# thomasgilgenast/hic3defdr

Measured on AMD Instinct MI355X. Metric: pixels/sec through estimate_disp+lrt, 4 reps @10kb; max-|Δq| vs reference, higher is better.
Workload: dtype f64; 1 GPU; cfg2: per GPU 1 chrom x 20000 bins, 4 reps (2+2), dist_thresh_max 250, estimate_disp (qcml) + lrt on HBM-resident inputs; disp_pixels_rank0=3757837, disp_pixels_total=3757837, parallelism=dp1 (chromosome shards; in-kernel Brent searches)

## Files before the change

hic3defdr_amd/csrc/h3d_api.hip:

```cpp
#include <hip/hip_runtime.h>
#include <hipcub/hipcub.hpp>

#include <algorithm>
#include <chrono>
#include <cstdarg>
#include <cstdio>
#include <cstdlib>
#include <cstring>
#include <map>
#include <string>
#include <thread>
#include <vector>

#include "h3d.h"
#include "h3d_ctx.h"
#include "h3d_errors.h"
#include "h3d_host.h"
#include "h3d_kernels.h"

using namespace h3d;
using namespace h3dint;
using h3derr::fail;

namespace h3dint {
// ... 137 lines not shown
}

}

namespace {

struct HostStamps {
  bool on = std::getenv("H3D_TIMING") != nullptr;
  std::chrono::steady_clock::time_point t0 = std::chrono::steady_clock::now();
  void operator()(const char* what) const {
    if (on)
      fprintf(stderr, "[h3d timing] %8.1f us %s\n",
              std::chrono::duration<double, std::micro>(
                  std::chrono::steady_clock::now() - t0).count(), what);
  }
};

template <typename K>
int resident_blocks(K kernel) {
  int nb = 0;
  if (hipOccupancyMaxActiveBlocksPerMultiprocessor(&nb, kernel, kBlock, 0) != hipSuccess ||
      nb < 1)
    nb = 1;
  return nb;
}

template <typename K>
int work_grid(h3d_ctx* ctx, K kernel, size_t max_items) {
  int& nb = ctx->resident[(const void*)kernel];
  if (nb == 0) nb = resident_blocks(kernel);
  return (int)std::max<size_t>(1, std::min<size_t>(max_items, (size_t)ctx->n_cu * nb));
}

template <int M, bool NLL>
void launch_disp_work(h3d_ctx* ctx, size_t max_items, const int32_t* raw_s,
                      const double* f_s, double* pd, int64_t n,
                      const int64_t* cs, const int32_t* cl, const int32_t* cd,
                      int C, const int32_t* rep_idx, const int32_t* n_rep,
                      const SegState* st, int* seg_flags, const int32_t* list,
                      int32_t* meta, double* partial) {
  {
    ProfScope ps(ctx, "disp_work", 0, 1);
#define H3D_EQ(WW)                                                                  \
  do {                                                                              \
    auto k = k_disp_work<M, WW, kEqualize, NLL>;                                    \
    hipLaunchKernelGGL(k, dim3(work_grid(ctx, k, max_items)), dim3(kBlock), 0,      \
                       ctx->stream, raw_s, f_s, pd, n, cs, cl, cd, C, rep_idx, n_rep, \
                       st, seg_flags, list, meta, partial, ctx->eq_static8);        \
  } while (0)
    if constexpr (M == 2 && NLL) {
      H3D_EQ(4);
    } else if constexpr (M == 2) {
      if (ctx->disp_w2 == 8) H3D_EQ(8);
      else if (ctx->disp_w2 == 6) H3D_EQ(6);
      else if (ctx->disp_w2 == 5) H3D_EQ(5);
      else H3D_EQ(4);
    } else if constexpr (M == 4) {
      if (ctx->disp_w == 4) H3D_EQ(4);
      else if (ctx->disp_w == 3) H3D_EQ(3);
      else if (ctx->disp_w == 2) H3D_EQ(2);
      else H3D_EQ(1);
    } else if constexpr (M == 8) {
      if (ctx->disp_w8 == 4) H3D_EQ(4);
      else H3D_EQ(1);
    } else {
      H3D_EQ(1);
    }
#undef H3D_EQ
  }
  if constexpr (NLL) {
    ProfScope ps(ctx, "disp_nll", 0);
    auto k = k_disp_work<M, 1, kNll>;
    if constexpr (M == 4) {
      if (ctx->nll_w == 2) k = k_disp_work<M, 2, kNll>;
      else if (ctx->nll_w == 4) k = k_disp_work<M, 4, kNll>;
    }
    hipLaunchKernelGGL(k, dim3(work_grid(ctx, k, max_items)), dim3(kBlock), 0,
                       ctx->stream, raw_s, f_s, pd, n, cs, cl, cd, C, rep_idx, n_rep,
                       st, seg_flags, list, meta, partial, ctx->eq_static8);
  }
}

template <int M>
void launch_brent(h3d_ctx* ctx, const double* pd, int64_t n, const int64_t* seg_start,
                  int S, int C, const int32_t* rep_idx, const int32_t* n_rep,
                  SegState* st, const int* seg_flags, double* result, int* queue,
                  const int32_t* gate_meta = nullptr, int live_min = 0,
                  const int* gang_abort = nullptr, bool queue_zeroed = false) {
  ProfScope ps(ctx, "disp_nll", 0);
  auto k = k_brent<M>;
  constexpr int kBrentBlock = brent_block<M>();
  const size_t lds_max = M <= 8 ? (size_t)ctx->brent_lds_kb * 1024 : 0;
  int& nb = ctx->resident[(const void*)k];
  if (nb == 0) {
    if (lds_max)
      (void)hipFuncSetAttribute((const void*)k, hipFuncAttributeMaxDynamicSharedMemorySize,
                                (int)lds_max);
    if (hipOccupancyMaxActiveBlocksPerMultiprocessor(&nb, k, kBrentBlock, lds_max) !=
            hipSuccess ||
        nb < 1)
      nb = 1;
  }
  const int grid = std::max(1, std::min(S, ctx->n_cu * nb));
  const size_t lds_bytes = M <= 8 ? (size_t)ctx->brent_lds_kb * 1024 : 0;
  const int64_t lds_px = (int64_t)(lds_bytes / (8 * (size_t)M));
  if (!queue_zeroed) (void)hipMemsetAsync(queue, 0, sizeof(int), ctx->stream);
  hipLaunchKernelGGL(k, dim3(grid), dim3(kBrentBlock), lds_px ? lds_px * 8 * M : 0,
                     ctx->stream, pd, n, seg_start, S, C, rep_idx, n_rep, st, seg_flags,
                     result, queue, ctx->work_count, lds_px, gate_meta, live_min, gang_abort);
#ifdef H3D_BRENT_CLOCK
  unsigned long long clk[38];
  (void)hipMemcpyFromSymbolAsync(clk, HIP_SYMBOL(g_brent_clk), sizeof(clk), 0,
                                 hipMemcpyDeviceToHost, ctx->stream);
  (void)hipStreamSynchronize(ctx->stream);
  fprintf(stderr, "[brent_clk] sum %llu bar1 %llu step %llu bar2 %llu stage %llu total %llu\n",
          clk[0], clk[1], clk[2], clk[3], clk[4], clk[5]);
  fprintf(stderr, "[brent_clk_wave] sum");
  for (int i = 0; i < 16; ++i) fprintf(stderr, " %llu", clk[6 + i]);
  fprintf(stderr, " bar1");
  for (int i = 0; i < 16; ++i) fprintf(stderr, " %llu", clk[22 + i]);
  fprintf(stderr, "\n");
#endif
}

struct GangTables {
  int32_t* task_seg = nullptr;
  int32_t* task_g = nullptr;
  int T = 0, gmax = 1, grid = 0;
  int64_t P = 0;
  double* part = nullptr;
  int* tag = nullptr;
  int* abort = nullptr;
  long long timeout = 0;
};

int gang_next_epoch(h3d_ctx* ctx, const GangTables& g, int S) {
  const size_t cap = ctx->bufs["gang_tag"].second;
  if (ctx->gang_tag_buf != (void*)g.tag || ctx->gang_tag_cap != cap ||
// ... 75 lines not shown
}

template <int M>
int gang_setup_dev(h3d_ctx* ctx, int64_t n, int D, int C, GangTables* g) {
  auto k = k_brent_gang<M>;
  int& nb = ctx->resident[(const void*)k];
  if (nb == 0) {
    if (hipOccupancyMaxActiveBlocksPerMultiprocessor(&nb, k, kGangThreads, 0) != hipSuccess ||
        nb < 1)
      nb = 1;
  }
  g->grid = ctx->n_cu * nb;
  const int64_t total = n * C;
  int64_t P = (total + 2 * (int64_t)g->grid - 1) / (2 * (int64_t)g->grid);
  P = std::max<int64_t>(P, (n + g->grid - 1) / g->grid);
  P = std::max<int64_t>(1024, (P + kGangThreads - 1) / kGangThreads * kGangThreads);
  if (ctx->gang_px > 0)
    P = std::max<int64_t>(std::max<int64_t>(64, ctx->gang_px), (n + g->grid - 1) / g->grid);
  g->P = P;
  g->gmax = (int)std::max<int64_t>(1, (n + P - 1) / P);
  g->T = (int)std::min<int64_t>(INT32_MAX, (int64_t)C * (g->gmax + D));
  const int S = D * C;
  g->task_seg = (int32_t*)scratch(ctx, "gang_seg", (size_t)g->T * 4);
  g->task_g = (int32_t*)scratch(ctx, "gang_g", (size_t)g->T * 4);
  g->part = (double*)scratch(ctx, "gang_part", (size_t)2 * S * g->gmax * 8);
  g->tag = (int*)scratch(ctx, "gang_tag", (size_t)2 * S * g->gmax * 4);
  g->abort = (int*)scratch(ctx, "gang_abort", 4);
  if (!g->task_seg || !g->task_g || !g->part || !g->tag || !g->abort)
    return fail(H3D_ENOMEM, "gang tables");
  g->timeout = gang_timeout(ctx);
  return 0;
}

template <int M>
void launch_brent_gang(h3d_ctx* ctx, const double* pd, int64_t n, const int64_t* seg_start,
                       int S, int C, const int32_t* rep_idx, const int32_t* n_rep,
                       SegState* st, const int* seg_flags, double* result, int* queue,
                       const GangTables& g, const int32_t* gate_meta = nullptr,
                       int live_max = 0, bool queue_zeroed = false) {
  ProfScope ps(ctx, "disp_nll", 0);
  if (!queue_zeroed) (void)hipMemsetAsync(queue, 0, sizeof(int), ctx->stream);
  const int epoch = gang_next_epoch(ctx, g, S);
  const int grid = std::max(1, std::min(g.T, g.grid));
  hipLaunchKernelGGL(k_brent_gang<M>, dim3(grid), dim3(kGangThreads), 0, ctx->stream, pd,
                     n, seg_start, S, C, rep_idx, n_rep, st, seg_flags, result, queue,
                     g.task_seg, g.task_g, g.T, g.P, g.part, g.tag, g.gmax, g.abort,
                     g.timeout, ctx->work_count, epoch, gate_meta, live_max);
}

int64_t disp_work_bytes(h3d_ctx* ctx, bool nll) {
  unsigned long long c[2] = {0, 0};
  if (!ctx->work_count) return 0;
  (void)hipMemcpyAsync(c, ctx->work_count, sizeof(c), hipMemcpyDeviceToHost, ctx->stream);
  (void)hipStreamSynchronize(ctx->stream);
  return nll ? (int64_t)(c[1] * 8ull) : (int64_t)(c[0] * 20ull);
}

}

extern "C" {

int h3d_version(void) { return 1; }

const char* h3d_last_error(void) { return h3derr::last(); }

int h3d_device_count(void) {
  int n = 0;
  if (hipGetDeviceCount(&n) != hipSuccess) return 0;
  return n;
}

h3d_ctx* h3d_open(int device) {
  int n = 0;
  if (hipGetDeviceCount(&n) != hipSuccess || n == 0) {
    fail(H3D_ENODEV, "no HIP device visible");
    return nullptr;
  }
// ... 5 lines not shown
  if (hipGetDeviceProperties(&prop, device) != hipSuccess) {
    fail(H3D_EHIP, "hipGetDeviceProperties failed");
    return nullptr;
  }
  if (std::strncmp(prop.gcnArchName, "gfx950", 6) != 0) {
    fail(H3D_ENODEV, "device %d is %s, libh3d is built for gfx950", device,
         prop.gcnArchName);
    return nullptr;
  }
  if (hipSetDevice(device) != hipSuccess) {
    fail(H3D_EHIP, "hipSetDevice failed");
    return nullptr;
  }
  h3d_ctx* ctx = new h3d_ctx();
  ctx->device = device;
  ctx->n_cu = prop.multiProcessorCount;
  if (hipStreamCreateWithFlags(&ctx->own, hipStreamNonBlocking) != hipSuccess) {
    delete ctx;
    fail(H3D_EHIP, "stream create failed");
    return nullptr;
  }
  ctx->stream = ctx->own;
  if (const char* e = std::getenv("H3D_DISP_W")) ctx->disp_w = std::atoi(e);
  if (const char* e = std::getenv("H3D_DISP_SORT")) ctx->disp_sort = std::atoi(e);
  if (const char* e = std::getenv("H3D_NLL_W")) ctx->nll_w = std::atoi(e);
  if (const char* e = std::getenv("H3D_DISP_W8")) ctx->disp_w8 = std::atoi(e);
  if (const char* e = std::getenv("H3D_DISP_W2")) ctx->disp_w2 = std::atoi(e);
  if (const char* e = std::getenv("H3D_PACK_GATHER")) ctx->pack_gather = std::atoi(e);
  if (const char* e = std::getenv("H3D_EQ_STATIC8"))
    ctx->eq_static8 = std::max(0, std::min(8, std::atoi(e)));
  if (const char* e = std::getenv("H3D_DISP_M2")) ctx->disp_m2 = std::atoi(e);
  if (const char* e = std::getenv("H3D_BRENT")) ctx->brent_gang = std::atoi(e);
  if (const char* e = std::getenv("H3D_BRENT_LDS_KB")) ctx->brent_lds_kb = std::atoi(e);
  if (const char* e = std::getenv("H3D_GANG_P")) ctx->gang_px = std::atoi(e);
  if (const char* e = std::getenv("H3D_DEV_SEG_TABLES")) ctx->dev_seg_tables = std::atoi(e);
  if (hipMalloc((void**)&ctx->work_count, 2 * sizeof(unsigned long long)) != hipSuccess ||
      hipMemset(ctx->work_count, 0, 2 * sizeof(unsigned long long)) != hipSuccess) {
    (void)hipStreamDestroy(ctx->own);
    delete ctx;
    fail(H3D_ENOMEM, "counter allocation failed");
    return nullptr;
  }
  return ctx;
}

void h3d_close(h3d_ctx* ctx) {
  if (!ctx) return;
  (void)hipSetDevice(ctx->device);
  (void)hipStreamSynchronize(ctx->stream);
  prof_collect(ctx);
  for (auto& kv : ctx->bufs)
    if (kv.second.first) (void)hipFree(kv.second.first);
  for (auto e : ctx->event_pool) (void)hipEventDestroy(e);
  if (ctx->work_count) (void)hipFree(ctx->work_count);
  if (ctx->h_meta) (void)hipHostFree(ctx->h_meta);
  if (ctx->h_stage) (void)hipHostFree(ctx->h_stage);
  if (ctx->h_res) (void)hipHostFree(ctx->h_res);
  if (ctx->h_stage_done) (void)hipEventDestroy(ctx->h_stage_done);
  if (ctx->bounce) (void)hipHostFree(ctx->bounce);
  if (ctx->bounce_ev) (void)hipEventDestroy(ctx->bounce_ev);
  if (ctx->land) (void)hipHostFree(ctx->land);
  if (ctx->own) (void)hipStreamDestroy(ctx->own);
  delete ctx;
}

int h3d_set_stream(h3d_ctx* ctx, void* stream) {
// ... 369 lines not shown
  HIP_TRY(hipMemcpyAsync(d_blob + up_lo, (char*)ctx->h_stage + up_lo, up_hi - up_lo,
                         hipMemcpyHostToDevice, s));
  HIP_TRY(hipEventRecord(ctx->h_stage_done, s));
  int64_t* d_cs = (int64_t*)(d_blob + parts[0].off);
  int32_t* d_cl = (int32_t*)(d_blob + parts[1].off);
  int32_t* d_cd = (int32_t*)(d_blob + parts[2].off);
  int32_t* d_scb = (int32_t*)(d_blob + parts[3].off);
  int32_t* d_sce = (int32_t*)(d_blob + parts[4].off);
  int32_t* d_nrep = (int32_t*)(d_blob + parts[5].off);
  int32_t* d_repidx = (int32_t*)(d_blob + parts[6].off);
  SegState* d_st = (SegState*)(d_blob + parts[7].off);
  int64_t* d_lpx = (int64_t*)(d_blob + parts[8].off);
  const size_t max_items = (size_t)std::max(n_chunks, 1) * C;
  int32_t* d_list = (int32_t*)scratch(ctx, "work_list", max_items * 4);
  int32_t* d_meta = (int32_t*)scratch(ctx, "work_meta", kWorkMetaInts * 4);
  int32_t* d_slb = (int32_t*)scratch(ctx, "seg_lb", S * 4);
  int32_t* d_sle = (int32_t*)scratch(ctx, "seg_le", S * 4);
  double* d_partial = (double*)scratch(ctx, "partial", max_items * 8 * kWavesPerBlock);
  double* d_total = (double*)scratch(ctx, "seg_total", S * 8);
  int* d_flags = (int*)scratch(ctx, "seg_flags", S * 4);
  double* d_res = (double*)scratch(ctx, "seg_result", S * 8);
  if (!d_cs || !d_cl || !d_cd || !d_scb || !d_sce || !d_nrep || !d_repidx ||
      !d_st || !d_lpx || !d_list || !d_meta || !d_slb || !d_sle || !d_partial ||
      !d_total || !d_flags || !d_res)
    return fail(H3D_ENOMEM, "disp scratch");
  if (!dev_tables) HIP_TRY(hipMemsetAsync(d_flags, 0, S * 4, s));
  int* d_bad = (int*)scratch(ctx, "dist_bad", 4);
  if (!d_bad) return fail(H3D_ENOMEM, "dist_bad");
  const int mslot = (maxnr <= 2 && ctx->disp_m2) ? 2
                    : maxnr <= 4                  ? 4
                    : maxnr <= 8                  ? 8
                    : maxnr <= 16                 ? 16
                                                  : 32;
  GangTables gang;
  const bool dual = dev_tables && !reduce && ctx->brent_gang == 1;
  if (dual) {
    const int grc = mslot == 2    ? gang_setup_dev<2>(ctx, n, D, C, &gang)
                    : mslot == 4  ? gang_setup_dev<4>(ctx, n, D, C, &gang)
                    : mslot == 8  ? gang_setup_dev<8>(ctx, n, D, C, &gang)
                    : mslot == 16 ? gang_setup_dev<16>(ctx, n, D, C, &gang)
                                  : gang_setup_dev<32>(ctx, n, D, C, &gang);
    if (grc) return grc;
  }
  if (dev_tables) {
    const int64_t* d_seg0 = (const int64_t*)scratch(ctx, "seg_start", (D + 1) * 8);
    hipLaunchKernelGGL(k_disp_tables, dim3(1), dim3(1024), 0, s, d_seg0, D, C, n, d_nrep,
                       d_cs, d_cl, d_cd, d_scb, d_sce, d_st, d_lpx, d_bad,
                       dual ? gang.P : (int64_t)1, dual ? gang.task_seg : nullptr,
                       dual ? gang.task_g : nullptr, ctx->qcml_tol, dual ? gang.T : 0,
                       d_flags, dual ? gang.abort : nullptr);
    dbg_launch("k_disp_tables");
  }
  stamp("tables uploaded");

  int* d_queue = (int*)scratch(ctx, "brent_queue", 2 * sizeof(int));
  if (!d_queue) return fail(H3D_ENOMEM, "brent queue");
  hipLaunchKernelGGL(k_seg_update, dim3(1), dim3(1024), 0, s, d_st, d_total,
                     d_flags, S, C, d_nrep, d_scb, d_sce, d_list, d_slb, d_sle,
                     d_res, d_meta, 1, 0, d_lpx, ctx->work_count, d_queue,
                     dual ? gang.P : (int64_t)1, dual ? gang.task_seg : nullptr,
                     dual ? gang.task_g : nullptr);
  if (!ctx->h_meta) HIP_TRY(hipHostMalloc((void**)&ctx->h_meta, 32, hipHostMallocDefault));
  int32_t* h_meta = ctx->h_meta;
  const size_t res_bytes = (size_t)S * 8 + (size_t)S * sizeof(SegState) + 8;
  if (ctx->h_res_bytes < res_bytes) {
    if (ctx->h_res) (void)hipHostFree(ctx->h_res);
    ctx->h_res = nullptr;
    ctx->h_res_bytes = 0;
    HIP_TRY(hipHostMalloc(&ctx->h_res, res_bytes, hipHostMallocDefault));
    ctx->h_res_bytes = res_bytes;
  }
  double* h_resd = (double*)ctx->h_res;
  SegState* h_sst = (SegState*)(h_resd + S);
  int* h_bad = (int*)(h_sst + S);
  *h_bad = 0;
  bool have_res = false;
  int rounds = 0, batch = 2, rc = 0;
  if (!reduce) {
    int64_t* d_seg = (int64_t*)scratch(ctx, "seg_start", (D + 1) * 8);
    if (!d_seg) return fail(H3D_ENOMEM, "brent scratch");
    if (n == 0) HIP_TRY(hipMemsetAsync(d_seg, 0, (D + 1) * 8, s));
    bool use_gang = ctx->brent_gang != 0 && n > 0 && !dev_tables;
    bool dual_on = dual;
    if (use_gang) {
      int grc = mslot == 2   ? gang_setup<2>(ctx, seg_start, D, C, &gang)
                : mslot == 4 ? gang_setup<4>(ctx, seg_start, D, C, &gang)
                : mslot == 8 ? gang_setup<8>(ctx, seg_start, D, C, &gang)
                : mslot == 16 ? gang_setup<16>(ctx, seg_start, D, C, &gang)
                              : gang_setup<32>(ctx, seg_start, D, C, &gang);
      if (grc == 1) use_gang = false;
      else if (grc) return grc;
    }
    batch = 5;
    while (true) {
      for (int b = 0; b < batch; ++b) {
#define H3D_QCML_ITER(MM)                                                                 \
  launch_disp_work<MM, false>(ctx, max_items, raw_s, f_s, pd, n, d_cs, d_cl, d_cd, C,     \
                              d_repidx, d_nrep, d_st, d_flags, d_list, d_meta, d_partial); \
  dbg_launch("equalize");                                                                 \
  if (dual_on) {                                                                          \
    launch_brent<MM>(ctx, pd, n, d_seg, S, C, d_repidx, d_nrep, d_st, d_flags, d_res,      \
                     d_queue, d_meta, ctx->n_cu, gang.abort, true);                        \
    dbg_launch("k_brent (dual)");                                                         \
    launch_brent_gang<MM>(ctx, pd, n, d_seg, S, C, d_repidx, d_nrep, d_st, d_flags, d_res, \
                          d_queue + 1, gang, d_meta, ctx->n_cu, true);                    \
    dbg_launch("k_brent_gang (dual)");                                                    \
  } else if (use_gang)                                                                    \
    launch_brent_gang<MM>(ctx, pd, n, d_seg, S, C, d_repidx, d_nrep, d_st, d_flags, d_res, \
                          d_queue + 1, gang, nullptr, 0, true);                           \
  else                                                                                    \
    launch_brent<MM>(ctx, pd, n, d_seg, S, C, d_repidx, d_nrep, d_st, d_flags, d_res,      \
                     d_queue, nullptr, 0, nullptr, true)
        dbg_launch("before qcml iteration");
        if (mslot == 2) { H3D_QCML_ITER(2); }
        else if (mslot == 4) { H3D_QCML_ITER(4); }
        else if (mslot == 8) { H3D_QCML_ITER(8); }
        else if (mslot == 16) { H3D_QCML_ITER(16); }
        else { H3D_QCML_ITER(32); }
#undef H3D_QCML_ITER
        {
          ProfScope ps(ctx, "disp_update", 0);
          hipLaunchKernelGGL(k_seg_update, dim3(1), dim3(1024), 0, s, d_st, d_total,
                             d_flags, S, C, d_nrep, d_scb, d_sce, d_list, d_slb, d_sle,
                             d_res, d_meta, 0, 0, d_lpx, ctx->work_count, d_queue,
                             dual_on ? gang.P : (int64_t)1,
                             dual_on ? gang.task_seg : nullptr,
                             dual_on ? gang.task_g : nullptr);
        }
        ++rounds;
      }
      hipEvent_t copied = ev_get(ctx);
      if (hipMemcpyAsync(h_meta, d_meta, 16, hipMemcpyDeviceToHost, s) != hipSuccess ||
          ((use_gang || dual_on) &&
           hipMemcpyAsync(h_meta + 4, gang.abort, 4, hipMemcpyDeviceToHost, s) != hipSuccess) ||
          hipMemcpyAsync(h_resd, d_res, (size_t)S * 8, hipMemcpyDeviceToHost, s) != hipSuccess ||
          hipMemcpyAsync(h_sst, d_st, (size_t)S * sizeof(SegState), hipMemcpyDeviceToHost, s) !=
              hipSuccess ||
          (dev_tables && hipMemcpyAsync(h_bad, d_bad, 4, hipMemcpyDeviceToHost, s) != hipSuccess) ||
          hipEventRecord(copied, s) != hipSuccess) {
        ctx->event_pool.push_back(copied);
        rc = fail(H3D_EHIP, "disp round copies failed: %s", hipGetErrorString(hipGetLastError()));
        break;
      }
      if (treq && D <= kTableMaxD) {
        rc = h3d_disp_tables_dev(ctx, d_res, D, C, treq->weighted, treq->frac, treq->aff,
                                 treq->d_tables);
        if (rc) {
          (void)hipEventSynchronize(copied);
          ctx->event_pool.push_back(copied);
          break;
        }
// ... 273 lines not shown
```

hic3defdr_amd/csrc/h3d_ctx.h:

```cpp
#pragma once

#include <hip/hip_runtime.h>

#include <cstdint>
#include <map>
#include <string>
#include <vector>

#include "h3d.h"
#include "h3d_errors.h"

#define HIP_TRY(expr)                                                      \
  do {                                                                     \
    hipError_t e_ = (expr);                                                \
    if (e_ != hipSuccess)                                                  \
      return h3derr::fail(H3D_EHIP, "%s failed: %s (%s:%d)", #expr,        \
                          hipGetErrorString(e_), __FILE__, __LINE__);      \
  } while (0)

namespace h3d {

struct PrepUnion {
  int R = 0, n_bins = 0;
  int64_t n_entries = 0, n_px = 0;
// ... 34 lines not shown
  hipStream_t stream = nullptr;
  int n_cu = 256;
  std::map<const void*, int> resident;
  int prof = 0;
  std::map<std::string, h3dint::ProfEntry> stats;
  std::vector<std::pair<std::string, std::pair<hipEvent_t, hipEvent_t>>> pending;
  std::vector<int64_t> pending_units;
  std::vector<hipEvent_t> event_pool;
  std::map<std::string, std::pair<void*, size_t>> bufs;
  h3d::PrepUnion prep;
  unsigned long long* work_count = nullptr;
  int32_t* h_meta = nullptr;
  void* h_stage = nullptr;
  size_t h_stage_bytes = 0;
  void* h_res = nullptr;
  size_t h_res_bytes = 0;
  hipEvent_t h_stage_done = nullptr;
  void* bounce = nullptr;
  size_t bounce_cap = 0, bounce_off = 0;
  hipEvent_t bounce_ev = nullptr;
  hipStream_t bounce_stream = nullptr;
  void* land = nullptr;
  size_t land_cap = 0;
  int disp_w = 4;
  int disp_sort = 2;
  int nll_w = 1;
  int disp_w2 = 4;
  int eq_static8 = 4;
  int pack_gather = 1;
  int disp_m2 = 1;
  int brent_gang = 1;
  int gang_aborts = 0;
  int brent_lds_kb = 128;
  double qcml_tol = 1e-4;
  int gang_px = 0;
  int gang_epoch = 0;
  void* gang_tag_buf = nullptr;
  size_t gang_tag_cap = 0;
  int last_S = 0;
  h3dint::TablePending tab_pending;
  int dev_seg_tables = 1;
  int disp_w8 = 4;
};

namespace h3dint {

constexpr int kLaunchBlock = 256;
constexpr int kTableMaxD = 1024;

void* scratch(h3d_ctx* ctx, const char* slot, size_t bytes);
void* scratch_keep(h3d_ctx* ctx, const char* slot, size_t bytes, size_t keep);
hipEvent_t ev_get(h3d_ctx* ctx);
int h2d_pinned(h3d_ctx* ctx, void* d_dst, const void* src, size_t bytes, hipStream_t s);
void* pinned_rd(h3d_ctx* ctx, size_t bytes);
int d2h_sync(h3d_ctx* ctx, void* dst, const void* d_src, size_t bytes, hipStream_t s);
void prof_collect(h3d_ctx* ctx);
int grid_for(h3d_ctx* ctx, int64_t n, int per_cu = 8);
int check_cond(const int32_t* cond_of_rep, int R, int C, std::vector<int>* nrep,
               std::vector<int32_t>* rep_idx);
int flags_to_code(int fl);
int table_status_copy(h3d_ctx* ctx, int* h_st);
int table_settle(h3d_ctx* ctx, const int* h_st);

struct ProfScope {
  h3d_ctx* ctx;
  const char* name;
// ... 23 lines not shown
```

hic3defdr_amd/csrc/h3d_kernels.h:

```cpp
#pragma once

#include <hip/hip_runtime.h>

#include <cstdint>

#include "h3d_model.h"

namespace h3d {

constexpr int kChunk = 256;
constexpr int kBlock = 256;
constexpr int kWavesPerBlock = kBlock / 64;
template <int M>
constexpr int brent_block() {
  return M >= 16 ? 512 : 1024;
}

__device__ inline double wave_sum(double v) {
#pragma unroll
  for (int off = 32; off > 0; off >>= 1) v += __shfl_xor(v, off, 64);
  return v;
}

__device__ inline double block_sum(double v, double* lds) {
// ... 283 lines not shown
        for (int j = 0; j < G; ++j) {
          task_seg[t0 + c * G + j] = d * C + c;
          task_g[t0 + c * G + j] = j;
        }
    }
    if (d < D) {
      scb[d] = b0;
      sce[d] = b0 + nch;
      const int64_t a = seg[d];
      for (int j = 0; j < nch; ++j) {
        cs[b0 + j] = a + (int64_t)j * kChunk;
        cl[b0 + j] = (int32_t)min((int64_t)kChunk, len - (int64_t)j * kChunk);
        cd[b0 + j] = d;
      }
      for (int c = 0; c < C; ++c) {
        seg_init(&st[d * C + c], (long long)len, n_rep[c], tol);
        lpx[d * C + c] = len;
      }
    }
    __syncthreads();
    if (threadIdx.x == 0) {
      s_carry += tot;
      s_tcarry += ttot;
    }
    __syncthreads();
  }
  if (task_seg)
    for (int t = s_tcarry + threadIdx.x; t < task_len; t += 1024) task_seg[t] = -1;
}

constexpr int kTaskHeadStride = 32;
constexpr int kWorkMetaInts = kTaskHeadStride * 17;

template <int M, int W, int PH, bool NLL = true>
__global__ __launch_bounds__(kBlock, W) void k_disp_work(
    const int32_t* __restrict__ raw_s, const double* __restrict__ f_s,
    double* __restrict__ pd, int64_t n, const int64_t* __restrict__ chunk_start,
    const int32_t* __restrict__ chunk_len, const int32_t* __restrict__ chunk_d,
    int C, const int32_t* __restrict__ rep_idx ,
    const int32_t* __restrict__ n_rep , const SegState* __restrict__ st,
    int* __restrict__ seg_flags, const int32_t* __restrict__ list,
    int32_t* __restrict__ meta ,
    double* __restrict__ partial, int static8) {
  const int beg = (PH == kEqualize) ? 0 : meta[2];
  const int end = (PH == kEqualize) ? meta[2] : meta[0];
  constexpr int kWv = kBlock / 64;
  const int lane = threadIdx.x & 63;
  const int64_t t0 = (int64_t)beg * kWv, t1 = (int64_t)end * kWv;
  const int64_t wt = (int64_t)gridDim.x * kWv;
  const int64_t tdyn = (t1 - t0 < 2 * wt) ? t1 : t0 + ((t1 - t0) / wt) * static8 / 8 * wt;
  const int64_t tl = t1 - tdyn;
  int32_t* heads = meta + kTaskHeadStride * (1 + (PH == kEqualize ? 0 : 8));
  const int grp = blockIdx.x & 7;
  unsigned spent = 0u;
  auto take = [&]() -> int64_t {
    if (tl <= 0) return t1;
#pragma unroll 1
    for (int k = 0; k < 8; ++k) {
      const int p = (grp + k) & 7;
      if ((spent >> p) & 1u) continue;
      const int64_t pb = tdyn + tl * p / 8, pe = tdyn + tl * (p + 1) / 8;
      int got = 0;
      if (lane == 0) got = atomicAdd(heads + kTaskHeadStride * p, 1);
      got = __shfl(got, 0, 64);
      if (pb + got < pe) return pb + got;
      spent |= 1u << p;
    }
    return t1;
  };
  __shared__ LogTab s_tab[kLogTabLen];
  for (int k = threadIdx.x; k < kLogTabLen; k += kBlock) s_tab[k] = kLogTab[k];
  __syncthreads();
  int64_t t = t0 + (int64_t)blockIdx.x * kWv + (threadIdx.x >> 6);
  if (t >= tdyn) t = take();
  for (; t < t1; t = (t + wt < tdyn) ? t + wt : take()) {
    const int w = (int)(t / kWv);
    const int q = (int)(t - (int64_t)w * kWv);
    const int item = list[w];
    const int chunk = item / C, c = item - chunk * C;
    const int s = chunk_d[chunk] * C + c;
    constexpr int phase = PH;
    const int nr = n_rep[c];
    double term = 0.0;
    const int i = q * 64 + lane;
    H3D_SEC_BEGIN(t_task);
    if (i < chunk_len[chunk] && nr < 8) {
      constexpr int MS = M < 8 ? M : 8;
      const int64_t px = chunk_start[chunk] + i;
      const NllConst kc = st[s].k;
      const int32_t* ri = rep_idx + c * kMaxReps;
      double lgsum = 0.0, z = 0.0;
      if (phase == kEqualize) {
        const double alpha = st[s].disp;
        double x[MS], f[MS], as[MS], lf[MS];
#pragma unroll
        for (int k = 0; k < MS; ++k) {
          const bool on = k < nr;
          x[k] = on ? (double)raw_s[(int64_t)ri[k] * n + px] : 0.0;
          f[k] = on ? f_s[(int64_t)ri[k] * n + px] : 1.0;
          lf[k] = on ? log_fast_checked(f[k], s_tab) : 0.0;
          as[k] = alpha;
        }
        int fl = 0;
        H3D_SEC_BEGIN(t_fit);
        const double f_mean = exp_fast(np_sum<MS>(lf, nr) / nr) - 0.0;
        const double mu = fit_mu<MS>(x, f, as, nr, ~0u, &fl, s_tab);
        H3D_SEC_END(0, t_fit);
        if (fl) atomicOr(&seg_flags[s], fl);
        const double mu_out0 = mu * f_mean;
        int fc = nr;
        unsigned up = 0u, lo = 0u;
#pragma unroll
        for (int k = MS - 1; k >= 0; --k)
          if (k < nr) {
            const double mi = mu * f[k];
// ... 311 lines not shown
      const int64_t j = i + (int64_t)q * kBlockT;
      on[q] = q == 0 || j < el - b;
#pragma unroll
      for (int k = 0; k < M; ++k) v[q][k] = (k < nr && on[q]) ? s_pd[k * lds_px + j] : 0.0;
    }
    double t[kPair];
#pragma unroll
    for (int q = 0; q < kPair; ++q) t[q] = term(v[q]);
#pragma unroll
    for (int q = 0; q < kPair; ++q)
      if (on[q]) acc += t[q];
  }
  for (int64_t px = el + threadIdx.x; px < e; px += kPair * kBlockT) {
    if constexpr (kPrio) brent_prio(lv, trip++, ntr);
    double v[kPair][M];
    bool on[kPair];
#pragma unroll
    for (int q = 0; q < kPair; ++q) {
      const int64_t qx = px + (int64_t)q * kBlockT;
      on[q] = q == 0 || qx < e;
#pragma unroll
      for (int k = 0; k < M; ++k) v[q][k] = (k < nr && on[q]) ? pd[(int64_t)ri[k] * n + qx] : 0.0;
    }
    double t[kPair];
#pragma unroll
    for (int q = 0; q < kPair; ++q) t[q] = term(v[q]);
#pragma unroll
    for (int q = 0; q < kPair; ++q)
      if (on[q]) acc += t[q];
  }
  return acc;
}

#ifdef H3D_BRENT_CLOCK
__device__ unsigned long long g_brent_clk[6 + 2 * 16];
#define H3D_BCLK(v) const long long v = clock64()
#define H3D_BADD(i, d) clk[i] += (unsigned long long)(d)
#else
#define H3D_BCLK(v)
#define H3D_BADD(i, d)
#endif

template <int M>
__global__ __launch_bounds__(brent_block<M>(), M >= 16 ? 2 : 4) void k_brent(
    const double* __restrict__ pd, int64_t n,
    const int64_t* __restrict__ seg_start , int S, int C,
    const int32_t* __restrict__ rep_idx ,
    const int32_t* __restrict__ n_rep , SegState* __restrict__ st,
    const int* __restrict__ seg_flags, double* __restrict__ result,
    int* __restrict__ queue, unsigned long long* __restrict__ work_count,
    int64_t lds_px, const int32_t* __restrict__ gate_meta, int live_min,
    const int* __restrict__ gang_abort) {
  extern __shared__ double s_pd[];
  if (gate_meta && gate_meta[3] < live_min && !(gang_abort && *gang_abort)) return;
  __shared__ SegState s_st;
  constexpr int kBrentBlock = brent_block<M>();
  __shared__ double wpart[kBrentBlock / 64];
  __shared__ int s_next, s_more;
  __shared__ LogTab s_tab[kLogTabLen];
  for (int t = threadIdx.x; t < kLogTabLen; t += kBrentBlock) s_tab[t] = kLogTab[t];
  const int lane = threadIdx.x & 63, wid = threadIdx.x >> 6;
#ifdef H3D_BRENT_CLOCK
  unsigned long long clk[6] = {0, 0, 0, 0, 0, 0};
  H3D_BCLK(k_t0);
#endif
  while (true) {
    __syncthreads();
    if (threadIdx.x == 0) s_next = atomicAdd(queue, 1);
    __syncthreads();
    const int s = s_next;
    if (s >= S) break;
    if (st[s].phase != kEqualize) continue;
    H3D_BCLK(c_stage0);
    if (threadIdx.x == 0) {
      s_st = st[s];
      s_st.flags |= seg_flags[s];
    }
    const int d = s / C, c = s - (s / C) * C;
    const int nr = n_rep[c];
    const int64_t b = seg_start[d], e = seg_start[d + 1];
    int ri[M];
#pragma unroll
    for (int k = 0; k < M; ++k) ri[k] = (k < nr) ? rep_idx[c * kMaxReps + k] : 0;
    const int64_t el = (e - b < lds_px) ? e : b + lds_px;
    for (int64_t i = threadIdx.x; i < el - b; i += kBrentBlock) {
#pragma unroll
      for (int k = 0; k < M; ++k)
        if (k < nr) s_pd[k * lds_px + i] = pd[(int64_t)ri[k] * n + b + i];
    }
    int evals = 0;
    __syncthreads();
    H3D_BCLK(c_stage1);
    H3D_BADD(4, c_stage1 - c_stage0);
    while (true) {
      H3D_BCLK(c0);
      const NllConst kc = s_st.k;
      constexpr bool kPr = H3D_BRENT_PRIO != 0;
      const double acc = (kc.r >= kNllLargeR)
          ? brent_segment_sum<M, kBrentBlock, 2, kPr>(s_pd, lds_px, pd, n, ri, nr, b, el, e, kc, s_tab)
          : (kc.r >= kNllMidR)
          ? brent_segment_sum<M, kBrentBlock, 1, kPr>(s_pd, lds_px, pd, n, ri, nr, b, el, e, kc, s_tab)
          : brent_segment_sum<M, kBrentBlock, 0, kPr>(s_pd, lds_px, pd, n, ri, nr, b, el, e, kc, s_tab);
      double wacc = acc;
#pragma unroll
      for (int off = 32; off > 0; off >>= 1) wacc += __shfl_xor(wacc, off, 64);
      if (lane == 0) wpart[wid] = wacc;
      H3D_BCLK(c1);
      __syncthreads();
      H3D_BCLK(c2);
      if (threadIdx.x == 0) {
        double total = 0.0;
#pragma unroll
        for (int w = 0; w < kBrentBlock / 64; ++w) total += wpart[w];
        seg_step_ool(&s_st, total, nr);
        s_more = (s_st.phase == kNll) ? 1 : 0;
      }
      H3D_BCLK(c3);
      ++evals;
      __syncthreads();
      H3D_BCLK(c4);
      H3D_BADD(0, c1 - c0);
      H3D_BADD(1, c2 - c1);
      H3D_BADD(2, c3 - c2);
      H3D_BADD(3, c4 - c3);
      if (!s_more) break;
    }
    if (threadIdx.x == 0) {
      s_st.last_evals = evals;
      st[s] = s_st;
      if (s_st.phase == kDone) result[s] = s_st.result;
      atomicAdd(&work_count[1], (unsigned long long)(e - b) * nr * evals);
    }
  }
#ifdef H3D_BRENT_CLOCK
  H3D_BCLK(k_t1);
  clk[5] = (unsigned long long)(k_t1 - k_t0);
  if (lane == 0) {
    for (int i = 0; i < 6; ++i) atomicAdd(&g_brent_clk[i], clk[i]);
    if (wid < 16) {
      atomicAdd(&g_brent_clk[6 + wid], clk[0]);
      atomicAdd(&g_brent_clk[22 + wid], clk[1]);
    }
  }
#endif
}

constexpr int kGangThreads = 256;

template <int M>
__global__ __launch_bounds__(kGangThreads) void k_brent_gang(
    const double* __restrict__ pd, int64_t n,
    const int64_t* __restrict__ seg_start , int S, int C,
    const int32_t* __restrict__ rep_idx ,
    const int32_t* __restrict__ n_rep , SegState* __restrict__ st,
    const int* __restrict__ seg_flags, double* __restrict__ result,
    int* __restrict__ queue, const int32_t* __restrict__ task_seg,
    const int32_t* __restrict__ task_g, int T, int64_t P,
    double* __restrict__ part , int* __restrict__ tag ,
    int gmax, int* __restrict__ abort_flag, long long timeout,
    unsigned long long* __restrict__ work_count, int epoch,
    const int32_t* __restrict__ gate_meta, int live_max) {
  if (gate_meta && (gate_meta[3] >= live_max || *abort_flag)) return;
  if (gate_meta && gate_meta[4] >= 0 && gate_meta[4] < T) T = gate_meta[4];
  __shared__ SegState s_st;
  __shared__ double wpart[kGangThreads / 64];
  __shared__ int s_next, s_more, s_abort;
  __shared__ LogTab s_tab[kLogTabLen];
  for (int t = threadIdx.x; t < kLogTabLen; t += kGangThreads) s_tab[t] = kLogTab[t];
  const int lane = threadIdx.x & 63, wid = threadIdx.x >> 6;
  while (true) {
    __syncthreads();
    if (threadIdx.x == 0) s_next = atomicAdd(queue, 1);
    __syncthreads();
    const int t = s_next;
    if (t >= T) break;
    const int s = task_seg[t], g = task_g[t];
    if (s < 0) continue;
    if (st[s].phase != kEqualize) continue;
    if (threadIdx.x == 0) {
      s_st = st[s];
      s_st.flags |= seg_flags[s];
      s_abort = 0;
    }
    const int d = s / C, c = s - (s / C) * C;
    const int nr = n_rep[c];
    const int64_t b = seg_start[d], e = seg_start[d + 1];
    const int G = (int)((e - b + P - 1) / P);
    const int64_t sb = b + (int64_t)g * P;
    const int64_t se = (sb + P < e) ? sb + P : e;
    int ri[M];
#pragma unroll
    for (int k = 0; k < M; ++k) ri[k] = (k < nr) ? rep_idx[c * kMaxReps + k] : 0;
    int evals = 0;
    __syncthreads();
    while (true) {
      const NllConst kc = s_st.k;
      double acc = (kc.r >= kNllLargeR)
          ? brent_segment_sum<M, kGangThreads, 2>(nullptr, 0, pd, n, ri, nr, sb, sb, se, kc, s_tab)
          : (kc.r >= kNllMidR)
          ? brent_segment_sum<M, kGangThreads, 1>(nullptr, 0, pd, n, ri, nr, sb, sb, se, kc, s_tab)
          : brent_segment_sum<M, kGangThreads, 0>(nullptr, 0, pd, n, ri, nr, sb, sb, se, kc, s_tab);
#pragma unroll
      for (int off = 32; off > 0; off >>= 1) acc += __shfl_xor(acc, off, 64);
      if (lane == 0) wpart[wid] = acc;
      __syncthreads();
      if (wid == 0) {
        double mine = 0.0;
#pragma unroll
        for (int w = 0; w < kGangThreads / 64; ++w) mine += wpart[w];
        double total = mine;
        bool ok = true;
        if (G > 1) {
          const size_t base = ((size_t)(evals & 1) * S + s) * gmax;
          const int want = (epoch << 10) | (evals + 1);
          if (lane == 0) {
            __hip_atomic_store(&part[base + g], mine, __ATOMIC_RELAXED,
                               __HIP_MEMORY_SCOPE_AGENT);
            __atomic_signal_fence(__ATOMIC_SEQ_CST);
            __builtin_amdgcn_s_waitcnt(0);
            __atomic_signal_fence(__ATOMIC_SEQ_CST);
            __hip_atomic_store(&tag[base + g], want, __ATOMIC_RELAXED,
                               __HIP_MEMORY_SCOPE_AGENT);
          }
          const long long t0 = wall_clock64();
          while (true) {
            bool mine_ready = true;
            for (int q = lane; q < G; q += 64)
              mine_ready &= __hip_atomic_load(&tag[base + q], __ATOMIC_RELAXED,
                                              __HIP_MEMORY_SCOPE_AGENT) == want;
            if (__all(mine_ready)) break;
            __builtin_amdgcn_s_sleep(1);
            const bool stop =
                __hip_atomic_load(abort_flag, __ATOMIC_RELAXED, __HIP_MEMORY_SCOPE_AGENT) ||
                wall_clock64() - t0 > timeout;
// ... 110 lines not shown
```

Baseline: 666.2 million pixels/s.

## Add full-replicate specialization of Brent NLL sums for two-rep conditions

```diff
diff --git a/hic3defdr_amd/csrc/h3d_api.hip b/hic3defdr_amd/csrc/h3d_api.hip
--- a/hic3defdr_amd/csrc/h3d_api.hip
+++ b/hic3defdr_amd/csrc/h3d_api.hip
@@ -193,7 +193,7 @@
   return (int)std::max<size_t>(1, std::min<size_t>(max_items, (size_t)ctx->n_cu * nb));
 }
 
-template <int M, bool NLL>
+template <int M, bool NLL, bool kFull = false>
 void launch_disp_work(h3d_ctx* ctx, size_t max_items, const int32_t* raw_s,
                       const double* f_s, double* pd, int64_t n,
                       const int64_t* cs, const int32_t* cl, const int32_t* cd,
@@ -204,7 +204,7 @@
     ProfScope ps(ctx, "disp_work", 0, 1);
 #define H3D_EQ(WW)                                                                  \
   do {                                                                              \
-    auto k = k_disp_work<M, WW, kEqualize, NLL>;                                    \
+    auto k = k_disp_work<M, WW, kEqualize, NLL, kFull>;                             \
     hipLaunchKernelGGL(k, dim3(work_grid(ctx, k, max_items)), dim3(kBlock), 0,      \
                        ctx->stream, raw_s, f_s, pd, n, cs, cl, cd, C, rep_idx, n_rep, \
                        st, seg_flags, list, meta, partial, ctx->eq_static8);        \
@@ -242,14 +242,14 @@
   }
 }
 
-template <int M>
+template <int M, bool kFull = false>
 void launch_brent(h3d_ctx* ctx, const double* pd, int64_t n, const int64_t* seg_start,
                   int S, int C, const int32_t* rep_idx, const int32_t* n_rep,
                   SegState* st, const int* seg_flags, double* result, int* queue,
                   const int32_t* gate_meta = nullptr, int live_min = 0,
                   const int* gang_abort = nullptr, bool queue_zeroed = false) {
   ProfScope ps(ctx, "disp_nll", 0);
-  auto k = k_brent<M>;
+  auto k = k_brent<M, kFull>;
   constexpr int kBrentBlock = brent_block<M>();
   const size_t lds_max = M <= 8 ? (size_t)ctx->brent_lds_kb * 1024 : 0;
   int& nb = ctx->resident[(const void*)k];
@@ -264,7 +264,8 @@
   }
   const int grid = std::max(1, std::min(S, ctx->n_cu * nb));
   const size_t lds_bytes = M <= 8 ? (size_t)ctx->brent_lds_kb * 1024 : 0;
-  const int64_t lds_px = (int64_t)(lds_bytes / (8 * (size_t)M));
+  const int64_t lds_px =
+      (int64_t)(lds_bytes / (8 * (size_t)M)) / kBrentBlock * kBrentBlock;
   if (!queue_zeroed) (void)hipMemsetAsync(queue, 0, sizeof(int), ctx->stream);
   hipLaunchKernelGGL(k, dim3(grid), dim3(kBrentBlock), lds_px ? lds_px * 8 * M : 0,
                      ctx->stream, pd, n, seg_start, S, C, rep_idx, n_rep, st, seg_flags,
@@ -406,7 +407,7 @@
   return 0;
 }
 
-template <int M>
+template <int M, bool kFull = false>
 void launch_brent_gang(h3d_ctx* ctx, const double* pd, int64_t n, const int64_t* seg_start,
                        int S, int C, const int32_t* rep_idx, const int32_t* n_rep,
                        SegState* st, const int* seg_flags, double* result, int* queue,
@@ -416,7 +417,16 @@
   if (!queue_zeroed) (void)hipMemsetAsync(queue, 0, sizeof(int), ctx->stream);
   const int epoch = gang_next_epoch(ctx, g, S);
   const int grid = std::max(1, std::min(g.T, g.grid));
-  hipLaunchKernelGGL(k_brent_gang<M>, dim3(grid), dim3(kGangThreads), 0, ctx->stream, pd,
+  auto k = k_brent_gang<M, kFull>;
+  if constexpr (kFull) {
+    int& nb = ctx->resident[(const void*)k];
+    if (nb == 0 &&
+        (hipOccupancyMaxActiveBlocksPerMultiprocessor(&nb, k, kGangThreads, 0) != hipSuccess ||
+         nb < 1))
+      nb = 1;
+    if (ctx->n_cu * nb < g.grid) k = k_brent_gang<M, false>;
+  }
+  hipLaunchKernelGGL(k, dim3(grid), dim3(kGangThreads), 0, ctx->stream, pd,
                      n, seg_start, S, C, rep_idx, n_rep, st, seg_flags, result, queue,
                      g.task_seg, g.task_g, g.T, g.P, g.part, g.tag, g.gmax, g.abort,
                      g.timeout, ctx->work_count, epoch, gate_meta, live_max);
@@ -488,6 +498,7 @@
   if (const char* e = std::getenv("H3D_DISP_M2")) ctx->disp_m2 = std::atoi(e);
   if (const char* e = std::getenv("H3D_BRENT")) ctx->brent_gang = std::atoi(e);
   if (const char* e = std::getenv("H3D_BRENT_LDS_KB")) ctx->brent_lds_kb = std::atoi(e);
+  if (const char* e = std::getenv("H3D_NLL_FULL")) ctx->nll_full = std::atoi(e);
   if (const char* e = std::getenv("H3D_GANG_P")) ctx->gang_px = std::atoi(e);
   if (const char* e = std::getenv("H3D_DEV_SEG_TABLES")) ctx->dev_seg_tables = std::atoi(e);
   if (hipMalloc((void**)&ctx->work_count, 2 * sizeof(unsigned long long)) != hipSuccess ||
@@ -923,6 +934,9 @@
                     : maxnr <= 8                  ? 8
                     : maxnr <= 16                 ? 16
                                                   : 32;
+  const bool nll_full =
+      ctx->nll_full && mslot == 2 &&
+      std::all_of(nrep.begin(), nrep.end(), [&](int r) { return r == mslot; });
   GangTables gang;
   const bool dual = dev_tables && !reduce && ctx->brent_gang == 1;
   if (dual) {
@@ -985,29 +999,31 @@
     batch = 5;
     while (true) {
       for (int b = 0; b < batch; ++b) {
-#define H3D_QCML_ITER(MM)                                                                 \
-  launch_disp_work<MM, false>(ctx, max_items, raw_s, f_s, pd, n, d_cs, d_cl, d_cd, C,     \
-                              d_repidx, d_nrep, d_st, d_flags, d_list, d_meta, d_partial); \
+#define H3D_QCML_ITER(MM, FF)                                                             \
+  launch_disp_work<MM, false, FF>(                                                        \
+      ctx, max_items, raw_s, f_s, pd, n, d_cs, d_cl, d_cd, C, d_repidx, d_nrep, d_st,     \
+      d_flags, d_list, d_meta, d_partial);                                                \
   dbg_launch("equalize");                                                                 \
   if (dual_on) {                                                                          \
-    launch_brent<MM>(ctx, pd, n, d_seg, S, C, d_repidx, d_nrep, d_st, d_flags, d_res,      \
-                     d_queue, d_meta, ctx->n_cu, gang.abort, true);                        \
+    launch_brent<MM, FF>(ctx, pd, n, d_seg, S, C, d_repidx, d_nrep, d_st, d_flags, d_res,  \
+                         d_queue, d_meta, ctx->n_cu, gang.abort, true);                    \
     dbg_launch("k_brent (dual)");                                                         \
-    launch_brent_gang<MM>(ctx, pd, n, d_seg, S, C, d_repidx, d_nrep, d_st, d_flags, d_res, \
-                          d_queue + 1, gang, d_meta, ctx->n_cu, true);                    \
+    launch_brent_gang<MM, FF>(ctx, pd, n, d_seg, S, C, d_repidx, d_nrep, d_st, d_flags,    \
+                              d_res, d_queue + 1, gang, d_meta, ctx->n_cu, true);         \
     dbg_launch("k_brent_gang (dual)");                                                    \
   } else if (use_gang)                                                                    \
-    launch_brent_gang<MM>(ctx, pd, n, d_seg, S, C, d_repidx, d_nrep, d_st, d_flags, d_res, \
-                          d_queue + 1, gang, nullptr, 0, true);                           \
+    launch_brent_gang<MM, FF>(ctx, pd, n, d_seg, S, C, d_repidx, d_nrep, d_st, d_flags,    \
+                              d_res, d_queue + 1, gang, nullptr, 0, true);                \
   else                                                                                    \
-    launch_brent<MM>(ctx, pd, n, d_seg, S, C, d_repidx, d_nrep, d_st, d_flags, d_res,      \
-                     d_queue, nullptr, 0, nullptr, true)
+    launch_brent<MM, FF>(ctx, pd, n, d_seg, S, C, d_repidx, d_nrep, d_st, d_flags, d_res,  \
+                         d_queue, nullptr, 0, nullptr, true)
         dbg_launch("before qcml iteration");
-        if (mslot == 2) { H3D_QCML_ITER(2); }
-        else if (mslot == 4) { H3D_QCML_ITER(4); }
-        else if (mslot == 8) { H3D_QCML_ITER(8); }
-        else if (mslot == 16) { H3D_QCML_ITER(16); }
-        else { H3D_QCML_ITER(32); }
+        if (mslot == 2 && nll_full) { H3D_QCML_ITER(2, true); }
+        else if (mslot == 2) { H3D_QCML_ITER(2, false); }
+        else if (mslot == 4) { H3D_QCML_ITER(4, false); }
+        else if (mslot == 8) { H3D_QCML_ITER(8, false); }
+        else if (mslot == 16) { H3D_QCML_ITER(16, false); }
+        else { H3D_QCML_ITER(32, false); }
 #undef H3D_QCML_ITER
         {
           ProfScope ps(ctx, "disp_update", 0);
diff --git a/hic3defdr_amd/csrc/h3d_ctx.h b/hic3defdr_amd/csrc/h3d_ctx.h
--- a/hic3defdr_amd/csrc/h3d_ctx.h
+++ b/hic3defdr_amd/csrc/h3d_ctx.h
@@ -90,6 +90,7 @@
   int brent_gang = 1;
   int gang_aborts = 0;
   int brent_lds_kb = 128;
+  int nll_full = 1;
   double qcml_tol = 1e-4;
   int gang_px = 0;
   int gang_epoch = 0;
diff --git a/hic3defdr_amd/csrc/h3d_kernels.h b/hic3defdr_amd/csrc/h3d_kernels.h
--- a/hic3defdr_amd/csrc/h3d_kernels.h
+++ b/hic3defdr_amd/csrc/h3d_kernels.h
@@ -339,7 +339,7 @@
 constexpr int kTaskHeadStride = 32;
 constexpr int kWorkMetaInts = kTaskHeadStride * 17;
 
-template <int M, int W, int PH, bool NLL = true>
+template <int M, int W, int PH, bool NLL = true, bool kFull = false>
 __global__ __launch_bounds__(kBlock, W) void k_disp_work(
     const int32_t* __restrict__ raw_s, const double* __restrict__ f_s,
     double* __restrict__ pd, int64_t n, const int64_t* __restrict__ chunk_start,
@@ -387,7 +387,7 @@
     const int chunk = item / C, c = item - chunk * C;
     const int s = chunk_d[chunk] * C + c;
     constexpr int phase = PH;
-    const int nr = n_rep[c];
+    const int nr = kFull ? M : n_rep[c];
     double term = 0.0;
     const int i = q * 64 + lane;
     H3D_SEC_BEGIN(t_task);
@@ -765,6 +765,137 @@
   return acc;
 }
 
+template <bool kPrio>
+struct BrentProgress {
+  int b1 = 0, b2 = 0, b3 = 0;
+  __device__ __forceinline__ explicit BrentProgress(int ntr) {
+    if constexpr (kPrio) {
+      const int m = max(ntr, 1), dv = H3D_BRENT_PRIO_DIV;
+      b1 = __builtin_amdgcn_readfirstlane((m + dv - 1) / dv);
+      b2 = __builtin_amdgcn_readfirstlane((2 * m + dv - 1) / dv);
+      b3 = __builtin_amdgcn_readfirstlane((3 * m + dv - 1) / dv);
+      __builtin_amdgcn_s_setprio(3);
+    }
+  }
+  __device__ __forceinline__ int next_after(int last) const {
+    if constexpr (kPrio) return last >= b3 ? INT_MAX : last >= b2 ? b3 : last >= b1 ? b2 : b1;
+    else return 0;
+  }
+  __device__ __forceinline__ void enter(int t, int& next) const {
+    if constexpr (kPrio) {
+      if (t >= next) {
+        if (t >= b3) {
+          __builtin_amdgcn_s_setprio(0);
+          next = INT_MAX;
+        } else if (t >= b2) {
+          __builtin_amdgcn_s_setprio(1);
+          next = b3;
+        } else {
+          __builtin_amdgcn_s_setprio(2);
+          next = b2;
+        }
+      }
+    }
+  }
+  __device__ __forceinline__ static int first_lane(int v) {
+    if constexpr (kPrio) return __builtin_amdgcn_readfirstlane(v);
+    else return 0;
+  }
+};
+
+template <int M, int kBlockT, int MODE, bool kPrio = false>
+__device__ __forceinline__ double brent_segment_sum_full(
+    const double* s_pd, int64_t lds_px, const double* __restrict__ pd, int64_t n,
+    const int* ri, int64_t b, int64_t el, int64_t e, const NllConst& kc,
+    const LogTab* s_tab) {
+  constexpr int kPair = kPair2<M>();
+  constexpr int kStep = kPair * kBlockT;
+  double acc = 0.0;
+  const BrentProgress<kPrio> pg((int)((e - b + kStep - 1) / kStep));
+  [[maybe_unused]] int done = 0;
+  auto term = [&](const double* v) {
+    if constexpr (MODE == 2) return nll_pixel_large<M>(v, M, kc, s_tab);
+    else if constexpr (MODE == 1) return nll_pixel_mid<M>(v, M, kc, s_tab);
+    else return nll_pixel<M>(v, M, kc, s_tab);
+  };
+  auto full_trips = [](int64_t len) {
+    const int64_t a = len - (int64_t)(kPair - 1) * kBlockT - (int64_t)threadIdx.x;
+    return a > 0 ? (int)((a + kStep - 1) / kStep) : 0;
+  };
+  auto one_trip = [&](auto full, auto&& ld, int64_t left) {
+    constexpr bool kAll = decltype(full)::value;
+    double v[kPair][M];
+    bool on[kPair];
+#pragma unroll
+    for (int q = 0; q < kPair; ++q) {
+      on[q] = kAll || q == 0 || (int64_t)q * kBlockT < left;
+#pragma unroll
+      for (int k = 0; k < M; ++k) v[q][k] = on[q] ? ld(q, k) : 0.0;
+    }
+    double t[kPair];
+#pragma unroll
+    for (int q = 0; q < kPair; ++q) t[q] = term(v[q]);
+#pragma unroll
+    for (int q = 0; q < kPair; ++q)
+      if (on[q]) acc += t[q];
+  };
+  const int64_t hl = el - b;
+  if (hl > 0) {
+    const double* h[M];
+#pragma unroll
+    for (int k = 0; k < M; ++k) h[k] = s_pd + k * lds_px + threadIdx.x;
+    auto ld = [&](int q, int k) { return h[k][q * kBlockT]; };
+    const int nf = full_trips(hl);
+    int next = pg.next_after(done - 1);
+    for (int t = 0; t < nf; ++t) {
+      pg.enter(done + t, next);
+      one_trip(std::true_type(), ld, 0);
+#pragma unroll
+      for (int k = 0; k < M; ++k) h[k] += kStep;
+    }
+    done += pg.first_lane(nf);
+    const int64_t left = hl - ((int64_t)threadIdx.x + (int64_t)nf * kStep);
+    if (pg.first_lane(left > 0)) {
+      next = pg.next_after(done - 1);
+      pg.enter(done++, next);
+    }
+    if (left > 0) one_trip(std::false_type(), ld, left);
+  }
+  const int64_t tl = e - el;
+  if (tl > 0) {
+    int64_t row[M];
+#pragma unroll
+    for (int k = 0; k < M; ++k) {
+      const uint64_t o = (uint64_t)((int64_t)ri[k] * n + el);
+      const uint32_t lo = __builtin_amdgcn_readfirstlane((uint32_t)o);
+      const uint32_t hi = __builtin_amdgcn_readfirstlane((uint32_t)(o >> 32));
+      row[k] = (int64_t)(((uint64_t)hi << 32) | lo);
+    }
+    const uint32_t lane_off = threadIdx.x * 8u;
+    int64_t adv = 0;
+    auto ld = [&](int q, int k) {
+      const char* p = (const char*)(pd + (row[k] + adv + q * kBlockT));
+      return *(const double*)(p + lane_off);
+    };
+    const int nf = full_trips(tl);
+    int next = pg.next_after(done - 1);
+    for (int t = 0; t < nf; ++t) {
+      pg.enter(done + t, next);
+      one_trip(std::true_type(), ld, 0);
+      adv += kStep;
+    }
+    done += pg.first_lane(nf);
+    adv = (int64_t)nf * kStep;
+    const int64_t left = tl - ((int64_t)threadIdx.x + adv);
+    if (pg.first_lane(left > 0)) {
+      next = pg.next_after(done - 1);
+      pg.enter(done++, next);
+    }
+    if (left > 0) one_trip(std::false_type(), ld, left);
+  }
+  return acc;
+}
+
 #ifdef H3D_BRENT_CLOCK
 __device__ unsigned long long g_brent_clk[6 + 2 * 16];
 #define H3D_BCLK(v) const long long v = clock64()
@@ -774,7 +905,8 @@
 #define H3D_BADD(i, d)
 #endif
 
-template <int M>
+
+template <int M, bool kFull = false>
 __global__ __launch_bounds__(brent_block<M>(), M >= 16 ? 2 : 4) void k_brent(
     const double* __restrict__ pd, int64_t n,
     const int64_t* __restrict__ seg_start , int S, int C,
@@ -810,7 +942,7 @@
       s_st.flags |= seg_flags[s];
     }
     const int d = s / C, c = s - (s / C) * C;
-    const int nr = n_rep[c];
+    const int nr = kFull ? M : n_rep[c];
     const int64_t b = seg_start[d], e = seg_start[d + 1];
     int ri[M];
 #pragma unroll
@@ -829,11 +961,20 @@
       H3D_BCLK(c0);
       const NllConst kc = s_st.k;
       constexpr bool kPr = H3D_BRENT_PRIO != 0;
-      const double acc = (kc.r >= kNllLargeR)
-          ? brent_segment_sum<M, kBrentBlock, 2, kPr>(s_pd, lds_px, pd, n, ri, nr, b, el, e, kc, s_tab)
-          : (kc.r >= kNllMidR)
-          ? brent_segment_sum<M, kBrentBlock, 1, kPr>(s_pd, lds_px, pd, n, ri, nr, b, el, e, kc, s_tab)
-          : brent_segment_sum<M, kBrentBlock, 0, kPr>(s_pd, lds_px, pd, n, ri, nr, b, el, e, kc, s_tab);
+      double acc;
+      if constexpr (kFull) {
+        acc = (kc.r >= kNllLargeR)
+            ? brent_segment_sum_full<M, kBrentBlock, 2, kPr>(s_pd, lds_px, pd, n, ri, b, el, e, kc, s_tab)
+            : (kc.r >= kNllMidR)
+            ? brent_segment_sum_full<M, kBrentBlock, 1, kPr>(s_pd, lds_px, pd, n, ri, b, el, e, kc, s_tab)
+            : brent_segment_sum_full<M, kBrentBlock, 0, kPr>(s_pd, lds_px, pd, n, ri, b, el, e, kc, s_tab);
+      } else {
+        acc = (kc.r >= kNllLargeR)
+            ? brent_segment_sum<M, kBrentBlock, 2, kPr>(s_pd, lds_px, pd, n, ri, nr, b, el, e, kc, s_tab)
+            : (kc.r >= kNllMidR)
+            ? brent_segment_sum<M, kBrentBlock, 1, kPr>(s_pd, lds_px, pd, n, ri, nr, b, el, e, kc, s_tab)
+            : brent_segment_sum<M, kBrentBlock, 0, kPr>(s_pd, lds_px, pd, n, ri, nr, b, el, e, kc, s_tab);
+      }
       double wacc = acc;
 #pragma unroll
       for (int off = 32; off > 0; off >>= 1) wacc += __shfl_xor(wacc, off, 64);
@@ -880,8 +1021,8 @@
 
 constexpr int kGangThreads = 256;
 
-template <int M>
-__global__ __launch_bounds__(kGangThreads) void k_brent_gang(
+template <int M, bool kFull = false>
+__global__ __launch_bounds__(kGangThreads, (kFull ? 4 : 0)) void k_brent_gang(
     const double* __restrict__ pd, int64_t n,
     const int64_t* __restrict__ seg_start , int S, int C,
     const int32_t* __restrict__ rep_idx ,
@@ -916,7 +1057,7 @@
       s_abort = 0;
     }
     const int d = s / C, c = s - (s / C) * C;
-    const int nr = n_rep[c];
+    const int nr = kFull ? M : n_rep[c];
     const int64_t b = seg_start[d], e = seg_start[d + 1];
     const int G = (int)((e - b + P - 1) / P);
     const int64_t sb = b + (int64_t)g * P;
@@ -928,11 +1069,20 @@
     __syncthreads();
     while (true) {
       const NllConst kc = s_st.k;
-      double acc = (kc.r >= kNllLargeR)
-          ? brent_segment_sum<M, kGangThreads, 2>(nullptr, 0, pd, n, ri, nr, sb, sb, se, kc, s_tab)
-          : (kc.r >= kNllMidR)
-          ? brent_segment_sum<M, kGangThreads, 1>(nullptr, 0, pd, n, ri, nr, sb, sb, se, kc, s_tab)
-          : brent_segment_sum<M, kGangThreads, 0>(nullptr, 0, pd, n, ri, nr, sb, sb, se, kc, s_tab);
+      double acc;
+      if constexpr (kFull) {
+        acc = (kc.r >= kNllLargeR)
+            ? brent_segment_sum_full<M, kGangThreads, 2>(nullptr, 0, pd, n, ri, sb, sb, se, kc, s_tab)
+            : (kc.r >= kNllMidR)
+            ? brent_segment_sum_full<M, kGangThreads, 1>(nullptr, 0, pd, n, ri, sb, sb, se, kc, s_tab)
+            : brent_segment_sum_full<M, kGangThreads, 0>(nullptr, 0, pd, n, ri, sb, sb, se, kc, s_tab);
+      } else {
+        acc = (kc.r >= kNllLargeR)
+            ? brent_segment_sum<M, kGangThreads, 2>(nullptr, 0, pd, n, ri, nr, sb, sb, se, kc, s_tab)
+            : (kc.r >= kNllMidR)
+            ? brent_segment_sum<M, kGangThreads, 1>(nullptr, 0, pd, n, ri, nr, sb, sb, se, kc, s_tab)
+            : brent_segment_sum<M, kGangThreads, 0>(nullptr, 0, pd, n, ri, nr, sb, sb, se, kc, s_tab);
+      }
 #pragma unroll
       for (int off = 32; off > 0; off >>= 1) acc += __shfl_xor(acc, off, 64);
       if (lane == 0) wpart[wid] = acc;
```

After: 705.4 million pixels/s, median of 6. 5.9% higher.
